# wenjunyang/xiangqi-alphazero

Measured on AMD Instinct MI355X. Metric: MCTS simulations/sec (whole node) + self-play games/hour, 256ch x 10blk ResNet, higher is better.
Workload: dtype f32

## Files before the change

xiangqi-alphazero_amd/csrc/xq_nn.hip:

```cpp
#include "xq_common.h"

namespace {

__global__ __launch_bounds__(64) void k_samples_to_batch(const xq_sample *__restrict__ rec, const int32_t *__restrict__ idx,
                                                         const uint8_t *__restrict__ flip, int n, double late_temperature,
                                                         double q_mix, float *__restrict__ states, float *__restrict__ pi,
                                                         float *__restrict__ z) {
    const int o = blockIdx.x;
    if (o >= n) return;
    const int lane = threadIdx.x;
    const xq_sample *s = rec + idx[o];
    const bool fl = flip[o] != 0;
    const int side = s->side;
    float *st = states + (size_t)o * XQ_STATE_FLOATS;
    for (int e = lane; e < XQ_STATE_FLOATS; e += 64) {
        const int plane = e / 90, sq = e - plane * 90;
        float v;
        if (plane == 14) {
            v = side == 1 ? 1.0f : 0.0f;
        } else {
            const int r = sq / 9, c = sq - r * 9;
            const int p = s->board[fl ? r * 9 + (8 - c) : sq];
            const int want = (plane < 7 ? plane + 1 : plane - 6) * (plane < 7 ? side : -side);
            v = p == want ? 1.0f : 0.0f;
        }
        st[e] = v;
    }
    float4 *p4 = (float4 *)(pi + (size_t)o * XQ_ACTION_SPACE);
    for (int i = lane; i < XQ_ACTION_SPACE / 4; i += 64) p4[i] = make_float4(0.f, 0.f, 0.f, 0.f);
    __syncthreads();
    const int m = s->n_moves;
    const double inv_t = s->late_temp ? 1.0 / late_temperature : 1.0;
    double total = 0.0;
    for (int i = 0; i < m; ++i) {
        const double c = (double)s->visits[i];
        total += s->late_temp ? (c > 0.0 ? pow(c, inv_t) : 0.0) : c;
    }
    for (int i = lane; i < m; i += 64) {
        const double c = (double)s->visits[i];
        const double w = s->late_temp ? (c > 0.0 ? pow(c, inv_t) : 0.0) : c;
        int a = s->actions[i];
        if (fl) {
            const int from = a / 90, to = a - from * 90;
            const int fr = from / 9, fc = from - fr * 9, tr = to / 9, tc = to - tr * 9;
            a = (fr * 9 + (8 - fc)) * 90 + tr * 9 + (8 - tc);
        }
        pi[(size_t)o * XQ_ACTION_SPACE + a] = total > 0.0 ? (float)(w / total) : 0.0f;
    }
    if (lane == 0) {
        const xq_sample_root_stats *rs = (const xq_sample_root_stats *)((const uint8_t *)s + XQ_SAMPLE_ROOT_STATS_OFFSET);
        float zv = (float)s->z;
        if (q_mix != 0.0 && rs->has_root_stats == 1) {
            const double a = (1.0 - q_mix) * (double)s->z, b = q_mix * (double)rs->root_q;
            zv = (float)(a + b);
        }
        z[o] = zv;
    }
}

__global__ __launch_bounds__(256) void k_bias_act(float4 *__restrict__ y, const float4 *__restrict__ bias,
                                                  const float4 *__restrict__ res, long long n4, int c4, int relu) {
    const long long stride = (long long)gridDim.x * blockDim.x;
    for (long long i = (long long)blockIdx.x * blockDim.x + threadIdx.x; i < n4; i += stride) {
        float4 v = y[i];
        const float4 b = bias[(int)(i % c4)];
        v.x += b.x; v.y += b.y; v.z += b.z; v.w += b.w;
        if (res) {
            const float4 r = res[i];
            v.x += r.x; v.y += r.y; v.z += r.z; v.w += r.w;
        }
        if (relu) {
            v.x = fmaxf(v.x, 0.0f); v.y = fmaxf(v.y, 0.0f); v.z = fmaxf(v.z, 0.0f); v.w = fmaxf(v.w, 0.0f);
        }
        y[i] = v;
    }
}


constexpr int HEAD_OUT = 36;
typedef float f32x2 __attribute__((ext_vector_type(2)));
__global__ __launch_bounds__(256) void k_heads_1x1(const float *__restrict__ H, const float *__restrict__ W,
                                                   const float *__restrict__ bias, float *__restrict__ P,
                                                   float *__restrict__ V, long long rows, int C,
                                                   const int32_t *__restrict__ live) {
    if (live) {
        const long long n = (long long)max(*live, 0) * 90;
        rows = n < rows ? n : rows;
    }
    extern __shared__ __attribute__((aligned(16))) char smem[];
    float *Ws = (float *)smem;
    for (int i = threadIdx.x * 4; i < HEAD_OUT * C; i += 256 * 4) *(float4 *)(Ws + i) = *(const float4 *)(W + i);
    __syncthreads();
    const int lane = threadIdx.x & 63, wave = threadIdx.x >> 6;
    const int r = lane >> 2, q = lane & 3;
    const int nk = C / 16;
    const long long n_batches = (rows + 15) / 16;
    for (long long bt = (long long)blockIdx.x * 4 + wave; bt < n_batches; bt += (long long)gridDim.x * 4) {
        const long long row = bt * 16 + r;
        const bool ok = row < rows;
        const float *hp = H + (ok ? row : 0) * C + 4 * q;
        f32x2 acc2[HEAD_OUT];
#pragma unroll
        for (int o = 0; o < HEAD_OUT; ++o) acc2[o] = f32x2{0.0f, 0.0f};
        float4 hv = *(const float4 *)hp;
        for (int k = 0; k < nk; ++k) {
            const f32x2 c01 = {hv.x, hv.y}, c23 = {hv.z, hv.w};
            if (k + 1 < nk) hv = *(const float4 *)(hp + 16 * (k + 1));
            const float *wk = Ws + 16 * k + 4 * q;
#pragma unroll
            for (int o = 0; o < HEAD_OUT; ++o) {
                const float4 w = *(const float4 *)(wk + o * C);
                acc2[o] = __builtin_elementwise_fma(c23, f32x2{w.z, w.w}, __builtin_elementwise_fma(c01, f32x2{w.x, w.y}, acc2[o]));
            }
        }
        float acc[HEAD_OUT];
#pragma unroll
        for (int o = 0; o < HEAD_OUT; ++o) {
            float v = acc2[o].x + acc2[o].y;
            v += __shfl_xor(v, 1);
            v += __shfl_xor(v, 2);
            acc[o] = fmaxf(v + bias[o], 0.0f);
        }
        if (ok) {
#pragma unroll
            for (int o = 0; o < HEAD_OUT; ++o) {
                if (o / 9 == q) {
                    if (o < 32) P[row * 32 + o] = acc[o];
                    else V[row * 4 + (o - 32)] = acc[o];
                }
            }
        }
    }
}


__global__ __launch_bounds__(256) void k_stem_conv(const float *__restrict__ X, const float *__restrict__ Wt,
                                                   const float *__restrict__ bias, float *__restrict__ Y, int C,
                                                   const int32_t *__restrict__ live) {
    __shared__ float xs[15 * 90];
    const int g = blockIdx.x, tid = threadIdx.x, lane = tid & 63, wave = tid >> 6;
    if (live && g >= *live) return;
    for (int i = tid; i < 15 * 90; i += 256) xs[i] = X[(size_t)g * (15 * 90) + i];
    __syncthreads();
    for (int pos = wave; pos < 90; pos += 4) {
        const int y = pos / 9, x = pos - y * 9;
        float xv[3];
        unsigned long long m[3];
#pragma unroll
        for (int r = 0; r < 3; ++r) {
            const int e = r * 64 + lane;
            float v = 0.0f;
            if (e < 135) {
                const int plane = e / 9, t = e - plane * 9, ty = t / 3, yy = y + ty - 1, xx = x + (t - ty * 3) - 1;
                if ((unsigned)yy < 10u && (unsigned)xx < 9u) v = xs[plane * 90 + yy * 9 + xx];
            }
            xv[r] = v;
            m[r] = __ballot(v != 0.0f);
        }
        for (int c0 = lane * 4; c0 < C; c0 += 256) {
            float4 acc = *(const float4 *)(bias + c0);
#pragma unroll
            for (int r = 0; r < 3; ++r) {
                unsigned long long mm = m[r];
                while (mm) {
                    const int b = __builtin_ctzll(mm);
                    mm &= mm - 1;
                    const float xe = __builtin_bit_cast(float, __builtin_amdgcn_readlane(__builtin_bit_cast(int, xv[r]), b));
                    const float4 w = *(const float4 *)(Wt + (size_t)(r * 64 + b) * C + c0);
                    acc.x = fmaf(xe, w.x, acc.x); acc.y = fmaf(xe, w.y, acc.y); acc.z = fmaf(xe, w.z, acc.z); acc.w = fmaf(xe, w.w, acc.w);
                }
            }
            acc.x = fmaxf(acc.x, 0.0f); acc.y = fmaxf(acc.y, 0.0f); acc.z = fmaxf(acc.z, 0.0f); acc.w = fmaxf(acc.w, 0.0f);
            *(float4 *)(Y + ((size_t)g * 90 + pos) * C + c0) = acc;
        }
    }
}


constexpr int PF4 = 2880 / 4;
__global__ __launch_bounds__(256) void k_policy_legal(const float *__restrict__ feat, const float *__restrict__ W,
                                                      const float *__restrict__ bias, const uint16_t *__restrict__ moves,
                                                      const int32_t *__restrict__ counts, int games, float *__restrict__ out,
                                                      const int32_t *__restrict__ live) {
    const int g = blockIdx.x * 4 + (int)(threadIdx.x >> 6);
    if (g >= games || (live && g >= *live)) return;
    const int lane = threadIdx.x & 63;
    int cnt = counts[g];
    cnt = cnt < 0 ? 0 : (cnt > XQ_MAXM ? XQ_MAXM : cnt);
    cnt = __builtin_amdgcn_readfirstlane(cnt);
    if (cnt == 0) return;
    const float4 *f4 = (const float4 *)(feat + (size_t)g * 2880);
    float4 f[12];
#pragma unroll
    for (int i = 0; i < 12; ++i) f[i] = (lane + 64 * i < PF4) ? f4[lane + 64 * i] : make_float4(0.f, 0.f, 0.f, 0.f);
    const uint16_t *mv = moves + (size_t)g * XQ_MAXM;
    float r0 = 0.0f, r1 = 0.0f;
    auto row_dot = [&](int a) __attribute__((always_inline)) {
        const float4 *w4 = (const float4 *)(W + (size_t)a * 2880);
        float4 w[12];
#pragma unroll
        for (int i = 0; i < 12; ++i) w[i] = (lane + 64 * i < PF4) ? w4[lane + 64 * i] : make_float4(0.f, 0.f, 0.f, 0.f);
        float s = 0.0f;
#pragma unroll
        for (int i = 0; i < 12; ++i) {
            s = fmaf(f[i].x, w[i].x, s); s = fmaf(f[i].y, w[i].y, s); s = fmaf(f[i].z, w[i].z, s); s = fmaf(f[i].w, w[i].w, s);
        }
        return s;
    };
    for (int m = 0; m < cnt; m += 2) {
        const int a0 = __builtin_amdgcn_readfirstlane((int)mv[m]);
        const int a1 = __builtin_amdgcn_readfirstlane((int)mv[m + 1 < cnt ? m + 1 : m]);
        float s0 = row_dot(a0), s1 = row_dot(a1);
#pragma unroll
        for (int off = 32; off > 0; off >>= 1) { s0 += __shfl_xor(s0, off); s1 += __shfl_xor(s1, off); }
        s0 += bias[a0]; s1 += bias[a1];
        if (m < 64) { if (lane == m) r0 = s0; if (lane == m + 1) r0 = s1; }
        else        { if (lane == m - 64) r1 = s0; if (lane == m - 63) r1 = s1; }
    }
    float *o = out + (size_t)g * XQ_MAXM;
    if (lane < cnt) o[lane] = r0;
    if (64 + lane < cnt) o[64 + lane] = r1;
}

constexpr int VGB = 4;
__global__ __launch_bounds__(128) void k_value_head(const float *__restrict__ vf, const float *__restrict__ w1t,
                                                    const float *__restrict__ b1, const float *__restrict__ w2,
                                                    const float *__restrict__ b2, int games, float *__restrict__ value,
                                                    const int32_t *__restrict__ live) {
    __shared__ __attribute__((aligned(16))) float vs[VGB][360];
    __shared__ float part[2][VGB];
    const int g0 = blockIdx.x * VGB, j = threadIdx.x;
    if (live) games = min(games, *live);
    if (g0 >= games) return;
    for (int i = j; i < VGB * 360; i += 128) {
        const int g = i / 360;
        vs[g][i - g * 360] = g0 + g < games ? vf[(size_t)(g0 + g) * 360 + (i - g * 360)] : 0.0f;
    }
    __syncthreads();
    float acc[VGB];
#pragma unroll
    for (int g = 0; g < VGB; ++g) acc[g] = 0.0f;
    for (int k = 0; k < 360; k += 4) {
        const float wa = w1t[(k + 0) * 128 + j], wb = w1t[(k + 1) * 128 + j], wc = w1t[(k + 2) * 128 + j], wd = w1t[(k + 3) * 128 + j];
#pragma unroll
        for (int g = 0; g < VGB; ++g) {
            const float4 v = *(const float4 *)&vs[g][k];
            acc[g] = fmaf(v.w, wd, fmaf(v.z, wc, fmaf(v.y, wb, fmaf(v.x, wa, acc[g]))));
        }
    }
    const float bj = b1[j], wj = w2[j];
#pragma unroll
    for (int g = 0; g < VGB; ++g) {
        float h = fmaxf(acc[g] + bj, 0.0f) * wj;
#pragma unroll
        for (int off = 32; off > 0; off >>= 1) h += __shfl_xor(h, off);
        if ((j & 63) == 0) part[j >> 6][g] = h;
    }
    __syncthreads();
    if (j < VGB && g0 + j < games) value[g0 + j] = tanhf(part[0][j] + part[1][j] + b2[0]);
}

}

extern "C" int xq_bias_act(float *dev_y, const float *dev_bias, const float *dev_residual, long long rows, int channels,
                           int relu, void *stream) {
    if (!dev_y || !dev_bias || rows < 0 || channels <= 0 || (channels & 3)) return XQ_ERR_ARG;
    if (((uintptr_t)dev_y | (uintptr_t)dev_bias | (uintptr_t)dev_residual) & 15) return XQ_ERR_ARG;
    const long long n4 = rows * (long long)(channels / 4);
    if (n4 == 0) return XQ_OK;
    long long blocks = (n4 + 255) / 256;
    if (blocks > 2048 * 4) blocks = 2048 * 4;
    hipLaunchKernelGGL(k_bias_act, dim3((unsigned)blocks), dim3(256), 0, (hipStream_t)stream, (float4 *)dev_y,
                       (const float4 *)dev_bias, (const float4 *)dev_residual, n4, channels / 4, relu);
    return xq::launch_status();
}

extern "C" int xq_samples_to_batch_ex(const void *dev_samples, const int32_t *dev_index, const uint8_t *dev_flip, int n,
                                      double late_temperature, const xq_batch_opts *opts, float *dev_states, float *dev_pi,
                                      float *dev_z, void *stream) {
    if (opts && (!(opts->q_mix >= 0.0 && opts->q_mix <= 1.0) || opts->reserved[0] != 0 || opts->reserved[1] != 0)) return XQ_ERR_ARG;
    if (n < 0 || (n > 0 && (!dev_samples || !dev_index || !dev_flip || !dev_states || !dev_pi || !dev_z))) return XQ_ERR_ARG;
    if (late_temperature <= 0.0 || ((uintptr_t)dev_pi & 15)) return XQ_ERR_ARG;
    if (n == 0) return XQ_OK;
    hipLaunchKernelGGL(k_samples_to_batch, dim3(n), dim3(64), 0, (hipStream_t)stream, (const xq_sample *)dev_samples, dev_index,
                       dev_flip, n, late_temperature, opts ? opts->q_mix : 0.0, dev_states, dev_pi, dev_z);
    return xq::launch_status();
}

extern "C" int xq_samples_to_batch(const void *dev_samples, const int32_t *dev_index, const uint8_t *dev_flip, int n,
                                   double late_temperature, float *dev_states, float *dev_pi, float *dev_z, void *stream) {
    return xq_samples_to_batch_ex(dev_samples, dev_index, dev_flip, n, late_temperature, nullptr, dev_states, dev_pi, dev_z, stream);
}

static int heads_1x1(const float *dev_h, const float *dev_w, const float *dev_bias, float *dev_p, float *dev_v, long long rows,
                     int channels, const int32_t *dev_live, void *stream) {
    if (!dev_h || !dev_w || !dev_bias || !dev_p || !dev_v || rows < 0 || channels < 16 || channels % 16 || channels > 1024) return XQ_ERR_ARG;
    if (((uintptr_t)dev_h | (uintptr_t)dev_w) & 15) return XQ_ERR_ARG;
    if (rows == 0) return XQ_OK;
    const int lds = HEAD_OUT * channels * 4;
    static thread_local int attr_lds = 0;
    if (lds > attr_lds) {
        XQ_TRY(hipFuncSetAttribute((const void *)k_heads_1x1, hipFuncAttributeMaxDynamicSharedMemorySize, lds));
        attr_lds = lds;
    }
    long long blocks = ((rows + 15) / 16 + 3) / 4;
    if (blocks > 256 * 8) blocks = 256 * 8;
    hipLaunchKernelGGL(k_heads_1x1, dim3((unsigned)blocks), dim3(256), lds, (hipStream_t)stream, dev_h, dev_w, dev_bias, dev_p,
                       dev_v, rows, channels, dev_live);
    return xq::launch_status();
}

extern "C" int xq_heads_1x1(const float *dev_h, const float *dev_w, const float *dev_bias, float *dev_p, float *dev_v,
                            long long rows, int channels, void *stream) {
    return heads_1x1(dev_h, dev_w, dev_bias, dev_p, dev_v, rows, channels, nullptr, stream);
}

extern "C" int xq_heads_1x1_live(const float *dev_h, const float *dev_w, const float *dev_bias, float *dev_p, float *dev_v,
                                 long long rows, const int32_t *dev_n, int channels, void *stream) {
    if (rows < 0) return XQ_ERR_ARG;
    if (rows == 0) return XQ_OK;
    if (!dev_n || rows % 90) return XQ_ERR_ARG;
    return heads_1x1(dev_h, dev_w, dev_bias, dev_p, dev_v, rows, channels, dev_n, stream);
}

static int stem_conv(const float *dev_planes, const float *dev_wt, const float *dev_bias, float *dev_y, int games, int channels,
                     const int32_t *dev_live, void *stream) {
    if (!dev_planes || !dev_wt || !dev_bias || !dev_y || games < 0 || channels < 4 || channels % 4) return XQ_ERR_ARG;
    if (((uintptr_t)dev_wt | (uintptr_t)dev_bias | (uintptr_t)dev_y) & 15) return XQ_ERR_ARG;
    if (games == 0) return XQ_OK;
    hipLaunchKernelGGL(k_stem_conv, dim3(games), dim3(256), 0, (hipStream_t)stream, dev_planes, dev_wt, dev_bias, dev_y, channels,
                       dev_live);
    return xq::launch_status();
}

extern "C" int xq_stem_conv(const float *dev_planes, const float *dev_wt, const float *dev_bias, float *dev_y, int games,
                            int channels, void *stream) {
    return stem_conv(dev_planes, dev_wt, dev_bias, dev_y, games, channels, nullptr, stream);
}

extern "C" int xq_stem_conv_live(const float *dev_planes, const float *dev_wt, const float *dev_bias, float *dev_y, int capacity,
                                 const int32_t *dev_n, int channels, void *stream) {
    if (capacity < 0) return XQ_ERR_ARG;
    if (capacity == 0) return XQ_OK;
    if (!dev_n) return XQ_ERR_ARG;
    return stem_conv(dev_planes, dev_wt, dev_bias, dev_y, capacity, channels, dev_n, stream);
}

static int policy_head_legal(const float *dev_feat, const float *dev_w, const float *dev_bias, const uint16_t *dev_moves,
                             const int32_t *dev_counts, int games, float *dev_out, const int32_t *dev_live, void *stream) {
    if (games < 0 || (games > 0 && (!dev_feat || !dev_w || !dev_bias || !dev_moves || !dev_counts || !dev_out))) return XQ_ERR_ARG;
    if (((uintptr_t)dev_feat | (uintptr_t)dev_w) & 15) return XQ_ERR_ARG;
    if (games == 0) return XQ_OK;
    hipLaunchKernelGGL(k_policy_legal, dim3((games + 3) / 4), dim3(256), 0, (hipStream_t)stream, dev_feat, dev_w, dev_bias, dev_moves,
                       dev_counts, games, dev_out, dev_live);
    return xq::launch_status();
}

extern "C" int xq_policy_head_legal(const float *dev_feat, const float *dev_w, const float *dev_bias, const uint16_t *dev_moves,
                                    const int32_t *dev_counts, int games, float *dev_out, void *stream) {
    return policy_head_legal(dev_feat, dev_w, dev_bias, dev_moves, dev_counts, games, dev_out, nullptr, stream);
}

extern "C" int xq_policy_head_legal_live(const float *dev_feat, const float *dev_w, const float *dev_bias, const uint16_t *dev_moves,
                                         const int32_t *dev_counts, int capacity, const int32_t *dev_n, float *dev_out, void *stream) {
    if (capacity < 0) return XQ_ERR_ARG;
    if (capacity == 0) return XQ_OK;
    if (!dev_n) return XQ_ERR_ARG;
    return policy_head_legal(dev_feat, dev_w, dev_bias, dev_moves, dev_counts, capacity, dev_out, dev_n, stream);
}

static int value_head(const float *dev_vfeat, const float *dev_w1t, const float *dev_b1, const float *dev_w2, const float *dev_b2,
                      int games, float *dev_value, const int32_t *dev_live, void *stream) {
    if (games < 0 || (games > 0 && (!dev_vfeat || !dev_w1t || !dev_b1 || !dev_w2 || !dev_b2 || !dev_value))) return XQ_ERR_ARG;
    if (games == 0) return XQ_OK;
    hipLaunchKernelGGL(k_value_head, dim3((games + VGB - 1) / VGB), dim3(128), 0, (hipStream_t)stream, dev_vfeat, dev_w1t, dev_b1,
                       dev_w2, dev_b2, games, dev_value, dev_live);
    return xq::launch_status();
}

extern "C" int xq_value_head(const float *dev_vfeat, const float *dev_w1t, const float *dev_b1, const float *dev_w2,
                             const float *dev_b2, int games, float *dev_value, void *stream) {
    return value_head(dev_vfeat, dev_w1t, dev_b1, dev_w2, dev_b2, games, dev_value, nullptr, stream);
}

extern "C" int xq_value_head_live(const float *dev_vfeat, const float *dev_w1t, const float *dev_b1, const float *dev_w2,
                                  const float *dev_b2, int capacity, const int32_t *dev_n, float *dev_value, void *stream) {
    if (capacity < 0) return XQ_ERR_ARG;
    if (capacity == 0) return XQ_OK;
    if (!dev_n) return XQ_ERR_ARG;
    return value_head(dev_vfeat, dev_w1t, dev_b1, dev_w2, dev_b2, capacity, dev_value, dev_n, stream);
}
```

Baseline: 160,000.

## Register-block heads 1x1 over two row tiles and compact nonzero lists in stem conv

The heads 1x1 kernel now processes two 16-row tiles per wave so each weight loaded from LDS is reused twice. It double-buffers weight loads in groups, prefetches input rows across chunk boundaries and into the next grid-stride batch, and caps the grid at a lower count with a two-blocks-per-SIMD launch bound. The stem conv pads the input planes in LDS so no bounds checks are needed, builds a per-wave compacted list of nonzero (value, weight offset) pairs instead of a readlane loop, consumes it in unrolled groups, and writes the output with nontemporal stores. The cost is higher register pressure in heads and extra LDS and bookkeeping in stem.

```diff
diff --git a/xiangqi-alphazero_amd/csrc/xq_nn.hip b/xiangqi-alphazero_amd/csrc/xq_nn.hip
--- a/xiangqi-alphazero_amd/csrc/xq_nn.hip
+++ b/xiangqi-alphazero_amd/csrc/xq_nn.hip
@@ -78,11 +78,62 @@
 
 
 constexpr int HEAD_OUT = 36;
+constexpr int HEAD_RB = 2;
+constexpr int HEAD_BATCH = 16 * HEAD_RB;
+constexpr int HEAD_PF = 4;
+constexpr int HEAD_WG = 4;
+#ifndef XQ_HEADS_GRID_CAP
+#define XQ_HEADS_GRID_CAP (256 * 4)
+#endif
 typedef float f32x2 __attribute__((ext_vector_type(2)));
-__global__ __launch_bounds__(256) void k_heads_1x1(const float *__restrict__ H, const float *__restrict__ W,
-                                                   const float *__restrict__ bias, float *__restrict__ P,
-                                                   float *__restrict__ V, long long rows, int C,
-                                                   const int32_t *__restrict__ live) {
+
+template <int PF>
+__device__ __forceinline__ void heads_chunks(f32x2 (&acc2)[HEAD_RB][HEAD_OUT], float4 (&hv)[HEAD_RB][PF],
+                                             const float *const (&fetch)[HEAD_RB], const float *wk, int C) {
+    static_assert(HEAD_OUT % HEAD_WG == 0, "whole groups");
+#pragma unroll
+    for (int d = 0; d < PF; ++d, wk += 16) {
+        float4 w[2][HEAD_WG];
+#pragma unroll
+        for (int j = 0; j < HEAD_WG; ++j) w[0][j] = *(const float4 *)(wk + j * C);
+#pragma unroll
+        for (int g = 0; g < HEAD_OUT / HEAD_WG; ++g) {
+            if (g + 1 < HEAD_OUT / HEAD_WG)
+#pragma unroll
+                for (int j = 0; j < HEAD_WG; ++j) w[(g + 1) & 1][j] = *(const float4 *)(wk + ((g + 1) * HEAD_WG + j) * C);
+#pragma unroll
+            for (int j = 0; j < HEAD_WG; ++j) {
+                const float4 wv = w[g & 1][j];
+                const int o = g * HEAD_WG + j;
+#pragma unroll
+                for (int i = 0; i < HEAD_RB; ++i)
+                    acc2[i][o] = __builtin_elementwise_fma(f32x2{hv[i][d].z, hv[i][d].w}, f32x2{wv.z, wv.w},
+                                                           __builtin_elementwise_fma(f32x2{hv[i][d].x, hv[i][d].y}, f32x2{wv.x, wv.y},
+                                                                                     acc2[i][o]));
+            }
+            __builtin_amdgcn_sched_barrier(0);
+        }
+#pragma unroll
+        for (int i = 0; i < HEAD_RB; ++i) hv[i][d] = *(const float4 *)(fetch[i] + 16 * d);
+        __builtin_amdgcn_sched_barrier(0);
+    }
+}
+
+__device__ __forceinline__ void heads_rows(long long bt, int r, int q, long long rows, int C, const float *__restrict__ H,
+                                           long long (&row)[HEAD_RB], bool (&ok)[HEAD_RB], const float *(&hp)[HEAD_RB]) {
+#pragma unroll
+    for (int i = 0; i < HEAD_RB; ++i) {
+        row[i] = bt * HEAD_BATCH + 16 * i + r;
+        ok[i] = row[i] < rows;
+        hp[i] = H + (ok[i] ? row[i] : 0) * C + 4 * q;
+    }
+}
+
+template <int PF>
+__global__ __launch_bounds__(256, 2) void k_heads_1x1(const float *__restrict__ H, const float *__restrict__ W,
+                                                      const float *__restrict__ bias, float *__restrict__ P,
+                                                      float *__restrict__ V, long long rows, int C,
+                                                      const int32_t *__restrict__ live) {
     if (live) {
         const long long n = (long long)max(*live, 0) * 90;
         rows = n < rows ? n : rows;
@@ -94,84 +145,168 @@
     const int lane = threadIdx.x & 63, wave = threadIdx.x >> 6;
     const int r = lane >> 2, q = lane & 3;
     const int nk = C / 16;
-    const long long n_batches = (rows + 15) / 16;
-    for (long long bt = (long long)blockIdx.x * 4 + wave; bt < n_batches; bt += (long long)gridDim.x * 4) {
-        const long long row = bt * 16 + r;
-        const bool ok = row < rows;
-        const float *hp = H + (ok ? row : 0) * C + 4 * q;
-        f32x2 acc2[HEAD_OUT];
-#pragma unroll
-        for (int o = 0; o < HEAD_OUT; ++o) acc2[o] = f32x2{0.0f, 0.0f};
-        float4 hv = *(const float4 *)hp;
-        for (int k = 0; k < nk; ++k) {
-            const f32x2 c01 = {hv.x, hv.y}, c23 = {hv.z, hv.w};
-            if (k + 1 < nk) hv = *(const float4 *)(hp + 16 * (k + 1));
-            const float *wk = Ws + 16 * k + 4 * q;
-#pragma unroll
-            for (int o = 0; o < HEAD_OUT; ++o) {
-                const float4 w = *(const float4 *)(wk + o * C);
-                acc2[o] = __builtin_elementwise_fma(c23, f32x2{w.z, w.w}, __builtin_elementwise_fma(c01, f32x2{w.x, w.y}, acc2[o]));
+    const long long n_batches = (rows + HEAD_BATCH - 1) / HEAD_BATCH, stride = (long long)gridDim.x * 4;
+    long long bt = (long long)blockIdx.x * 4 + wave;
+    if (bt >= n_batches) return;
+    long long row[HEAD_RB];
+    bool ok[HEAD_RB];
+    const float *hp[HEAD_RB];
+    heads_rows(bt, r, q, rows, C, H, row, ok, hp);
+    float4 hv[HEAD_RB][PF];
+#pragma unroll
+    for (int d = 0; d < PF; ++d) {
+#pragma unroll
+        for (int i = 0; i < HEAD_RB; ++i) hv[i][d] = *(const float4 *)(hp[i] + 16 * d);
+        __builtin_amdgcn_sched_barrier(0);
+    }
+    for (; bt < n_batches; bt += stride) {
+        long long row_n[HEAD_RB];
+        bool ok_n[HEAD_RB];
+        const float *hp_n[HEAD_RB];
+        heads_rows(bt + stride < n_batches ? bt + stride : bt, r, q, rows, C, H, row_n, ok_n, hp_n);
+        f32x2 acc2[HEAD_RB][HEAD_OUT];
+#pragma unroll
+        for (int i = 0; i < HEAD_RB; ++i)
+#pragma unroll
+            for (int o = 0; o < HEAD_OUT; ++o) acc2[i][o] = f32x2{0.0f, 0.0f};
+        for (int k0 = 0; k0 < nk; k0 += PF) {
+            const float *fetch[HEAD_RB];
+#pragma unroll
+            for (int i = 0; i < HEAD_RB; ++i) fetch[i] = k0 + PF < nk ? hp[i] + 16 * (k0 + PF) : hp_n[i];
+            heads_chunks<PF>(acc2, hv, fetch, Ws + 4 * q + 16 * k0, C);
+        }
+#pragma unroll
+        for (int i = 0; i < HEAD_RB; ++i) {
+#pragma unroll
+            for (int qq = 0; qq < 4; ++qq) {
+                float acc[9];
+#pragma unroll
+                for (int j = 0; j < 9; ++j) {
+                    const int o = 9 * qq + j;
+                    float v = acc2[i][o].x + acc2[i][o].y;
+                    v += __shfl_xor(v, 1);
+                    v += __shfl_xor(v, 2);
+                    acc[j] = fmaxf(v + bias[o], 0.0f);
+                }
+                if (ok[i] && q == qq) {
+#pragma unroll
+                    for (int j = 0; j < 9; ++j) {
+                        const int o = 9 * qq + j;
+                        if (o < 32) P[row[i] * 32 + o] = acc[j];
+                        else V[row[i] * 4 + (o - 32)] = acc[j];
+                    }
+                }
+                __builtin_amdgcn_sched_barrier(0);
             }
         }
-        float acc[HEAD_OUT];
-#pragma unroll
-        for (int o = 0; o < HEAD_OUT; ++o) {
-            float v = acc2[o].x + acc2[o].y;
-            v += __shfl_xor(v, 1);
-            v += __shfl_xor(v, 2);
-            acc[o] = fmaxf(v + bias[o], 0.0f);
-        }
-        if (ok) {
-#pragma unroll
-            for (int o = 0; o < HEAD_OUT; ++o) {
-                if (o / 9 == q) {
-                    if (o < 32) P[row * 32 + o] = acc[o];
-                    else V[row * 4 + (o - 32)] = acc[o];
-                }
-            }
-        }
-    }
-}
-
+#pragma unroll
+        for (int i = 0; i < HEAD_RB; ++i) { row[i] = row_n[i]; ok[i] = ok_n[i]; hp[i] = hp_n[i]; }
+    }
+}
+
+
+#ifndef XQ_STEM_GROUP
+#define XQ_STEM_GROUP 8
+#endif
+constexpr int STEM_GROUP = XQ_STEM_GROUP;
+constexpr int STEM_LIST = 136;
+constexpr int STEM_PW = 11, STEM_PP = 12 * STEM_PW;
+typedef float f32x4 __attribute__((ext_vector_type(4)));
+
+template <int N>
+__device__ __forceinline__ void stem_group(const uint2 *lst, int i, const char *__restrict__ wp, unsigned c0b, float4 &acc) {
+    float xe[N];
+    unsigned off[N];
+    float4 w[N];
+    if constexpr (N >= 2) {
+#pragma unroll
+        for (int j = 0; j < N; j += 2) {
+            const uint4 a = *(const uint4 *)(lst + i + j);
+            xe[j] = __builtin_bit_cast(float, a.x); off[j] = a.y;
+            xe[j + 1] = __builtin_bit_cast(float, a.z); off[j + 1] = a.w;
+        }
+    } else {
+        const uint2 a = lst[i];
+        xe[0] = __builtin_bit_cast(float, a.x); off[0] = a.y;
+    }
+#pragma unroll
+    for (int j = 0; j < N; ++j) {
+#ifdef XQ_STEM_ABL_ONE_ENTRY
+        asm volatile("v_mov_b32 %0, 0" : "=v"(off[j]));
+#endif
+        w[j] = *(const float4 *)(wp + (off[j] + c0b));
+    }
+#pragma unroll
+    for (int j = 0; j < N; ++j) {
+        acc.x = fmaf(xe[j], w[j].x, acc.x); acc.y = fmaf(xe[j], w[j].y, acc.y);
+        acc.z = fmaf(xe[j], w[j].z, acc.z); acc.w = fmaf(xe[j], w[j].w, acc.w);
+    }
+}
+
+template <int N>
+__device__ __forceinline__ void stem_tail(int n, int i, const uint2 *lst, const char *__restrict__ wp, unsigned c0b, float4 &acc) {
+    if constexpr (N >= 1) {
+        if (n & N) {
+            stem_group<N>(lst, i, wp, c0b, acc);
+            i += N;
+        }
+        stem_tail<N / 2>(n, i, lst, wp, c0b, acc);
+    }
+}
 
 __global__ __launch_bounds__(256) void k_stem_conv(const float *__restrict__ X, const float *__restrict__ Wt,
                                                    const float *__restrict__ bias, float *__restrict__ Y, int C,
                                                    const int32_t *__restrict__ live) {
-    __shared__ float xs[15 * 90];
-    const int g = blockIdx.x, tid = threadIdx.x, lane = tid & 63, wave = tid >> 6;
+    __shared__ float xs[16 * STEM_PP];
+    __shared__ __attribute__((aligned(16))) uint2 lsts[4][STEM_LIST];
+    const int g = blockIdx.x, tid = threadIdx.x, lane = tid & 63, wave = __builtin_amdgcn_readfirstlane(tid >> 6);
     if (live && g >= *live) return;
-    for (int i = tid; i < 15 * 90; i += 256) xs[i] = X[(size_t)g * (15 * 90) + i];
+    {
+        constexpr int PER = (16 * STEM_PP + 255) / 256;
+        float t[PER];
+#pragma unroll
+        for (int j = 0; j < PER; ++j) {
+            const int i = tid + 256 * j, plane = i / STEM_PP, rr = i - plane * STEM_PP, py = rr / STEM_PW, px = rr - py * STEM_PW;
+            const bool board = plane < 15 && py >= 1 && py <= 10 && px >= 1 && px <= 9;
+            t[j] = board ? X[(size_t)g * (15 * 90) + plane * 90 + (py - 1) * 9 + (px - 1)] : 0.0f;
+        }
+#pragma unroll
+        for (int j = 0; j < PER; ++j)
+            if (tid + 256 * j < 16 * STEM_PP) xs[tid + 256 * j] = t[j];
+    }
     __syncthreads();
+    int xoff[3];
+    unsigned woff[3];
+#pragma unroll
+    for (int r = 0; r < 3; ++r) {
+        const int e = r * 64 + lane, plane = e / 9, t = e - plane * 9, ty = t / 3;
+        xoff[r] = e < 135 ? plane * STEM_PP + ty * STEM_PW + (t - ty * 3) : 15 * STEM_PP;
+        woff[r] = (unsigned)e * (unsigned)C * 4u;
+    }
+    uint2 *lst = lsts[wave];
+    const unsigned cb = (unsigned)C * 4u;
     for (int pos = wave; pos < 90; pos += 4) {
-        const int y = pos / 9, x = pos - y * 9;
-        float xv[3];
-        unsigned long long m[3];
+        const int y = pos / 9, poff = y * STEM_PW + (pos - y * 9);
+        int n_set = 0;
 #pragma unroll
         for (int r = 0; r < 3; ++r) {
-            const int e = r * 64 + lane;
-            float v = 0.0f;
-            if (e < 135) {
-                const int plane = e / 9, t = e - plane * 9, ty = t / 3, yy = y + ty - 1, xx = x + (t - ty * 3) - 1;
-                if ((unsigned)yy < 10u && (unsigned)xx < 9u) v = xs[plane * 90 + yy * 9 + xx];
+            const float v = xs[xoff[r] + poff];
+            const unsigned long long m = __ballot(v != 0.0f);
+            if (v != 0.0f) {
+                const int rank = n_set + __builtin_amdgcn_mbcnt_hi((unsigned)(m >> 32), __builtin_amdgcn_mbcnt_lo((unsigned)m, 0));
+                lst[rank] = make_uint2(__builtin_bit_cast(unsigned, v), woff[r]);
             }
-            xv[r] = v;
-            m[r] = __ballot(v != 0.0f);
-        }
-        for (int c0 = lane * 4; c0 < C; c0 += 256) {
-            float4 acc = *(const float4 *)(bias + c0);
-#pragma unroll
-            for (int r = 0; r < 3; ++r) {
-                unsigned long long mm = m[r];
-                while (mm) {
-                    const int b = __builtin_ctzll(mm);
-                    mm &= mm - 1;
-                    const float xe = __builtin_bit_cast(float, __builtin_amdgcn_readlane(__builtin_bit_cast(int, xv[r]), b));
-                    const float4 w = *(const float4 *)(Wt + (size_t)(r * 64 + b) * C + c0);
-                    acc.x = fmaf(xe, w.x, acc.x); acc.y = fmaf(xe, w.y, acc.y); acc.z = fmaf(xe, w.z, acc.z); acc.w = fmaf(xe, w.w, acc.w);
-                }
-            }
+            n_set += __builtin_popcountll(m);
+        }
+        char *yp = (char *)(Y + ((size_t)g * 90 + pos) * C);
+        for (unsigned c0b = lane * 16; c0b < cb; c0b += 1024) {
+            float4 acc = *(const float4 *)((const char *)bias + c0b);
+            int i = 0;
+            for (; i + STEM_GROUP <= n_set; i += STEM_GROUP) stem_group<STEM_GROUP>(lst, i, (const char *)Wt, c0b, acc);
+            stem_tail<STEM_GROUP / 2>(n_set, i, lst, (const char *)Wt, c0b, acc);
             acc.x = fmaxf(acc.x, 0.0f); acc.y = fmaxf(acc.y, 0.0f); acc.z = fmaxf(acc.z, 0.0f); acc.w = fmaxf(acc.w, 0.0f);
-            *(float4 *)(Y + ((size_t)g * 90 + pos) * C + c0) = acc;
+            const f32x4 out = {acc.x, acc.y, acc.z, acc.w};
+            __builtin_nontemporal_store(out, (f32x4 *)(yp + c0b));
         }
     }
 }
@@ -298,15 +433,17 @@
     if (((uintptr_t)dev_h | (uintptr_t)dev_w) & 15) return XQ_ERR_ARG;
     if (rows == 0) return XQ_OK;
     const int lds = HEAD_OUT * channels * 4;
-    static thread_local int attr_lds = 0;
-    if (lds > attr_lds) {
-        XQ_TRY(hipFuncSetAttribute((const void *)k_heads_1x1, hipFuncAttributeMaxDynamicSharedMemorySize, lds));
-        attr_lds = lds;
-    }
-    long long blocks = ((rows + 15) / 16 + 3) / 4;
-    if (blocks > 256 * 8) blocks = 256 * 8;
-    hipLaunchKernelGGL(k_heads_1x1, dim3((unsigned)blocks), dim3(256), lds, (hipStream_t)stream, dev_h, dev_w, dev_bias, dev_p,
-                       dev_v, rows, channels, dev_live);
+    const bool ring = channels % (16 * HEAD_PF) == 0;
+    const auto kernel = ring ? k_heads_1x1<HEAD_PF> : k_heads_1x1<1>;
+    static thread_local int attr_lds[2] = {0, 0};
+    if (lds > attr_lds[ring]) {
+        XQ_TRY(hipFuncSetAttribute((const void *)kernel, hipFuncAttributeMaxDynamicSharedMemorySize, lds));
+        attr_lds[ring] = lds;
+    }
+    long long blocks = ((rows + HEAD_BATCH - 1) / HEAD_BATCH + 3) / 4;
+    if (blocks > XQ_HEADS_GRID_CAP) blocks = XQ_HEADS_GRID_CAP;
+    hipLaunchKernelGGL(kernel, dim3((unsigned)blocks), dim3(256), lds, (hipStream_t)stream, dev_h, dev_w, dev_bias, dev_p, dev_v,
+                       rows, channels, dev_live);
     return xq::launch_status();
 }
 
```

New measurement: 160,400 (median of 6 runs). Within noise of the previous version (+0.2%).
